# graphdeco-inria/reduced-3dgs

Hardware: AMD Instinct MI355X
Metric: train iters/s (fwd+bwd) + Mpix/s render, 500k Gaussians @1600x1062 (higher is better)
Workload: dtype f32

## Files before the change

include/r3dgs_rasterizer.h:

```cpp
#ifndef R3DGS_RASTERIZER_H
#define R3DGS_RASTERIZER_H

#include <stddef.h>
#include <stdint.h>

#ifdef __cplusplus
extern "C" {
#endif

typedef char* (*r3dgs_alloc_fn)(size_t bytes, void* user);

const char* r3dgs_version(void);

const char* r3dgs_last_error(void);

size_t r3dgs_geometry_bytes(int P);
size_t r3dgs_geometry_bytes_lean(int P);
size_t r3dgs_binning_bytes(int P, int width, int height, int reserve);
size_t r3dgs_image_bytes(int width, int height);
int r3dgs_binning_capacity(int P, int width, int height, size_t bytes);

int r3dgs_mark_visible(int P, const float* means3D, const float* viewmatrix, const float* projmatrix,
                       unsigned char* present, void* stream);

// ... 17 lines not shown
                            int prefiltered, float* out_color, int* out_touched_pixels, float* out_transmittance,
                            int* radii, int calculate_mean_transmittance, int debug, void* stream);

#define R3DGS_PASS_TRUNCATED 1
#define R3DGS_PASS_DEPTH_BUCKET_OVERFLOW 2
int r3dgs_reserve_hint(int P, int width, int height);
int r3dgs_reserve_hint_view(int P, int width, int height, const float* viewmatrix);
long long r3dgs_forward_reserved(char* geom_buffer, char* binning_buffer, char* image_buffer, int reserve, int P,
                                 const int* D, int M, const float* background, int width, int height,
                                 const float* means3D, const float* shs, const float* colors_precomp,
                                 const float* opacities, const float* scales, float scale_modifier,
                                 const float* rotations, const float* cov3D_precomp, const float* viewmatrix,
                                 const float* projmatrix, const float* cam_pos, float tan_fovx, float tan_fovy,
                                 int prefiltered, float* out_color, int* out_touched_pixels, float* out_transmittance,
                                 int* radii, int calculate_mean_transmittance, int debug, void* stream);
long long r3dgs_inference_forward_reserved(char* geom_buffer, char* binning_buffer, char* image_buffer, int reserve,
                                           int P, const int* D, int bandsNum, const int* coeffsNum,
                                           const int* perBandPrimitiveCount, const int* cumSumPrimitiveCount,
                                           const float* background, int width, int height, const float* means3D,
                                           const float* shs, const float* colors_precomp, const float* opacities,
                                           const float* scales, float scale_modifier, const float* rotations,
                                           const float* cov3D_precomp, const float* viewmatrix, const float* projmatrix,
                                           const float* cam_pos, float tan_fovx, float tan_fovy, int prefiltered,
                                           float* out_color, int* out_touched_pixels, float* out_transmittance,
                                           int* radii, int calculate_mean_transmittance, int debug, void* stream);
int r3dgs_pass_query(long long ticket, int wait, int* num_rendered, int* visible, int* reserve, int* flags);
long long r3dgs_reserve_overflow_events(int* last_num_rendered, int* last_reserve);
int r3dgs_pass_pairs(long long ticket, int wait);
int r3dgs_forward_pairs(void);
int r3dgs_set_tight_rects(int on);
int r3dgs_export_rects(int P, char* geom_buffer, unsigned short* rects, void* stream);

int r3dgs_set_tile_order(int on);
int r3dgs_set_sh_cache(int on);
int r3dgs_set_f64_chain(int on);
void r3dgs_forward_hint(int will_backward);

int r3dgs_set_bwd_segments(int on);

int r3dgs_export_tile_order(int P, int R, int width, int height, char* binning_buffer, char* image_buffer,
                            unsigned int* quad_depth, unsigned int* unit_order, void* stream);
int r3dgs_bwd_units_cap(int R, int width, int height);

void r3dgs_reserve_forget(void);
void r3dgs_reserve_forget_view(const float* viewmatrix);

int r3dgs_backward(int P, const int* D, int M, int R, const float* background, int width, int height,
                   const float* means3D, const float* shs, const float* colors_precomp, const float* scales,
                   float scale_modifier, const float* rotations, const float* cov3D_precomp,
                   const float* viewmatrix, const float* projmatrix, const float* campos, float tan_fovx,
                   float tan_fovy, const int* radii, char* geom_buffer, char* binning_buffer, char* image_buffer,
                   const float* dL_dpix, float* dL_dmean2D, float* dL_dconic, float* dL_dopacity, float* dL_dcolor,
                   float* dL_dmean3D, float* dL_dcov3D, float* dL_dsh, float* dL_dscale, float* dL_drot,
                   float lambda_sh_sparsity, int debug, void* stream);

int r3dgs_forward_params(r3dgs_alloc_fn geometryBuffer, void* geometry_user, r3dgs_alloc_fn binningBuffer,
                         void* binning_user, r3dgs_alloc_fn imageBuffer, void* image_user, int P, const int* D, int M,
                         const float* background, int width, int height, const float* means3D, const float* features_dc,
                         const float* features_rest, const float* opacities, const float* scaling_raw,
                         float scale_modifier, const float* rotation_raw, const float* viewmatrix, const float* projmatrix,
                         const float* cam_pos, float tan_fovx, float tan_fovy, int prefiltered, float* out_color,
                         int* out_touched_pixels, float* out_transmittance, int* radii, int calculate_mean_transmittance,
                         int debug, void* stream);
long long r3dgs_forward_params_reserved(char* geom_buffer, char* binning_buffer, char* image_buffer, int reserve, int P,
                                        const int* D, int M, const float* background, int width, int height,
                                        const float* means3D, const float* features_dc, const float* features_rest,
// ... 36 lines not shown
```

reduced-3dgs_amd/csrc/binning.hip:

```cpp
#include <cstdlib>
#include <cstring>
#include <mutex>
#include <string>

#include <rocprim/rocprim.hpp>

#include "depth_sort.h"

namespace r3 {

struct GatherTiles {
    const uint32_t* tiles;
    __host__ __device__ uint32_t operator()(uint32_t id) const { return tiles[id]; }
};

size_t depth_sort_temp_bytes(size_t P)
{
    size_t a = 0, b = 0;
    uint32_t* n = nullptr;
    R3_HIP(rocprim::radix_sort_pairs(nullptr, a, n, n, rocprim::counting_iterator<uint32_t>(0), n, P, 0, 32));
    auto it = rocprim::make_transform_iterator(n, GatherTiles{n});
    R3_HIP(rocprim::inclusive_scan(nullptr, b, it, n, P, rocprim::plus<uint32_t>()));
    return (a > b ? a : b) + 256;
}
// ... 253 lines not shown
__global__ __launch_bounds__(256) void radix_digit_scan_kernel(const RadixArgs* __restrict__ ap)
{
    __shared__ uint32_t s_sum[256];
    const RadixArgs a = *ap;
    const uint32_t nb = (a.hdr->num_pairs + (uint32_t)kRadixBlock - 1u) / (uint32_t)kRadixBlock;
    const uint32_t* row = a.rows + (size_t)blockIdx.x * a.row_stride;
    uint32_t* out = a.base + (size_t)blockIdx.x * a.row_stride;
    uint32_t run = 0;
    for (uint32_t c0 = 0; c0 < nb; c0 += 1024u) {
        const uint32_t i = c0 + threadIdx.x * 4u;
        uint4 v = make_uint4(0u, 0u, 0u, 0u);
        if (i < nb) v = *reinterpret_cast<const uint4*>(row + i);
        if (i + 1 >= nb) v.y = 0u;
        if (i + 2 >= nb) v.z = 0u;
        if (i + 3 >= nb) v.w = 0u;
        const uint32_t mine = v.x + v.y + v.z + v.w;
        const uint32_t incl = block256_inclusive_scan(mine, s_sum);
        const uint32_t b0 = run + incl - mine;
        if (i < nb) *reinterpret_cast<uint4*>(out + i) = make_uint4(b0, b0 + v.x, b0 + v.x + v.y, b0 + v.x + v.y + v.z);
        run += s_sum[0] + s_sum[1] + s_sum[2] + s_sum[3];
    }
    if (threadIdx.x == 0) a.total[blockIdx.x] = run;
}

template <class IO, int BITS>
__device__ __forceinline__ void radix_scatter_block(const RadixArgs& a, uint32_t R, uint32_t blk_id)
{
    constexpr int kWaves = 4, kRounds = kRadixBlock / 256, kBins = 1 << BITS;
    __shared__ uint32_t s_wcount[kWaves][kBins];
    __shared__ uint32_t s_start[kBins];
    __shared__ uint32_t s_off[kWaves][kBins];
    __shared__ uint32_t s_delta[kBins];
    __shared__ typename IO::Reg s_keys[kRadixBlock];
    typedef typename IO::Reg Word;
    const int shift = a.shift;
    const int lane = threadIdx.x & 63, w = threadIdx.x >> 6;
    for (int t = threadIdx.x; t < kWaves * kBins; t += 256) (&s_wcount[0][0])[t] = 0;
    if (w == 0) {
        constexpr int kPer = kBins / 64;
        uint32_t v[kPer], sum = 0;
#pragma unroll
        for (int k = 0; k < kPer; k++) {
            v[k] = a.total[kPer * lane + k];
            sum += v[k];
        }
        uint32_t incl = sum;
        for (int off = 1; off < 64; off <<= 1) {
            const uint32_t up = (uint32_t)__shfl_up((int)incl, off);
            if (lane >= off) incl += up;
        }
        uint32_t run = incl - sum;
#pragma unroll
        for (int k = 0; k < kPer; k++) {
            s_start[kPer * lane + k] = run;
            run += v[k];
        }
    }
    __syncthreads();
    const uint32_t blk = blk_id * (uint32_t)kRadixBlock + (uint32_t)w * (kRadixBlock / kWaves);
    Word key[kRounds];
    uint32_t lrank[kRounds];
#pragma unroll
    for (int r = 0; r < kRounds; r++) {
        const uint32_t i = blk + r * 64u + lane;
        key[r] = i < R ? IO::load(a.in, a.cap, i) : (Word)0;
    }
// ... 19 lines not shown
            v[k] = s_wcount[0][d] + s_wcount[1][d] + s_wcount[2][d] + s_wcount[3][d];
            sum += v[k];
        }
        uint32_t incl = sum;
        for (int off = 1; off < 64; off <<= 1) {
            const uint32_t up = (uint32_t)__shfl_up((int)incl, off);
            if (lane >= off) incl += up;
        }
        uint32_t run = incl - sum;
#pragma unroll
        for (int k = 0; k < kPer; k++) {
            const int d = kPer * lane + k;
            s_delta[d] = s_start[d] + a.base[(size_t)d * a.row_stride + blk_id] - run;
            uint32_t r2 = run;
#pragma unroll
            for (int q = 0; q < kWaves; q++) {
                s_off[q][d] = r2;
                r2 += s_wcount[q][d];
            }
            run += v[k];
        }
    }
    __syncthreads();
#pragma unroll
    for (int r = 0; r < kRounds; r++) {
        if (blk + r * 64u + lane < R) {
            const uint32_t d = (uint32_t)(key[r] >> shift) & (uint32_t)(kBins - 1);
            s_keys[s_off[w][d] + lrank[r]] = key[r];
        }
    }
    __syncthreads();
    const uint32_t base0 = blk_id * (uint32_t)kRadixBlock;
    const uint32_t nvalid = min((uint32_t)kRadixBlock, R - base0);
#pragma unroll
    for (int r = 0; r < kRounds; r++) {
        const uint32_t i = (uint32_t)r * 256u + threadIdx.x;
        if (i < nvalid) {
            const Word k = s_keys[i];
            const uint32_t d = (uint32_t)(k >> shift) & (uint32_t)(kBins - 1);
            IO::store(a.out, a.ids_out, a.cap, i + s_delta[d], k);
        }
    }
}

template <class IO, int BITS>
__global__ __launch_bounds__(256) void radix_scatter_kernel(const RadixArgs* __restrict__ ap)
{
    const RadixArgs a = *ap;
    const uint32_t R = a.hdr->num_pairs;
    for (uint32_t blk = blockIdx.x; blk * (uint32_t)kRadixBlock < R; blk += gridDim.x) {
        radix_scatter_block<IO, BITS>(a, R, blk);
        __syncthreads();
    }
}

template <class IO>
__global__ __launch_bounds__(256) void tile_ranges_kernel(const RangesArgs* __restrict__ ap)
{
    typedef typename IO::Reg Word;
    const RangesArgs a = *ap;
    const int R = (int)a.hdr->num_pairs;
  for (int blk = (int)blockIdx.x; blk * 1024 < R; blk += (int)gridDim.x) {
    const int i0 = (blk * 256 + threadIdx.x) * 4;
    if (i0 >= R) continue;
    unsigned char* __restrict__ pair_flag = a.pair_flag;
    uint32_t* __restrict__ point_list = a.point_list;
    uint2* ranges = a.ranges;
    const int rank_bits = a.rank_bits;
    if (i0 + 4 <= R)
        *reinterpret_cast<uint32_t*>(pair_flag + i0) = 0u;
    else
        for (int k = i0; k < R; k++) pair_flag[k] = 0;
    const int n = min(4, R - i0);
    uint32_t tile[4];
// ... 15 lines not shown
    }
    uint32_t prev = i0 ? IO::tile_at(a.sorted, a.cap, (uint32_t)(i0 - 1), rank_bits) : 0xFFFFFFFFu;
    for (int k = 0; k < n; k++) {
        const uint32_t cur = tile[k];
        const int i = i0 + k;
        if (i == 0)
            ranges[cur].x = 0;
        else if (cur != prev) {
            ranges[prev].y = i;
            ranges[cur].x = i;
        }
        if (i == R - 1) ranges[cur].y = R;
        prev = cur;
    }
  }
}

template <class IO>
static void issue_tile_binning_t(const FwdPlan& p, const FwdPassArgs* a, hipStream_t s)
{
    const PairLayout& l = p.layout;
    const uint32_t nbk = (p.grid_pairs + (uint32_t)kRadixBlock - 1u) / (uint32_t)kRadixBlock;
    const int bins = 1 << l.digit_bits;
    hipLaunchKernelGGL(emit_pairs_kernel<IO>, dim3(nbk), dim3(256), 0, s, &a->emit);
    for (int k = 0; k < l.passes; k++) {
        const RadixArgs* ra = &a->radix[k];
        if (k > 0) hipLaunchKernelGGL(radix_hist_kernel<IO>, dim3(nbk), dim3(256), 0, s, ra);
        hipLaunchKernelGGL(radix_digit_scan_kernel, dim3(bins), dim3(256), 0, s, ra);
        if (l.digit_bits == 7)
            hipLaunchKernelGGL((radix_scatter_kernel<IO, 7>), dim3(nbk), dim3(256), 0, s, ra);
        else
            hipLaunchKernelGGL((radix_scatter_kernel<IO, 8>), dim3(nbk), dim3(256), 0, s, ra);
    }
    hipLaunchKernelGGL(tile_ranges_kernel<IO>, dim3((p.grid_pairs + 1023u) / 1024u), dim3(256), 0, s, &a->ranges);
}

void issue_tile_binning(const FwdPlan& p, const FwdPassArgs* a, hipStream_t s)
{
    if (p.layout.wide == 2)
        issue_tile_binning_t<IoSplit>(p, a, s);
    else if (p.layout.wide == 1)
        issue_tile_binning_t<IoWide>(p, a, s);
    else
        issue_tile_binning_t<IoNarrow>(p, a, s);
}

template <class IO>
__global__ __launch_bounds__(256) void export_keys_kernel(int R, uint32_t cap, int rank_bits, const char* __restrict__ sorted,
                                                          const uint32_t* __restrict__ point_list,
                                                          const uint32_t* __restrict__ depth_key, const GeomHeader* hdr,
                                                          uint64_t* keys)
{
    const int i = blockIdx.x * 256 + threadIdx.x;
    if (i >= R) return;
    if ((uint32_t)i >= hdr->num_pairs) {
        keys[i] = ~(uint64_t)0;
        return;
    }
    keys[i] = ((uint64_t)IO::tile_at(sorted, cap, (uint32_t)i, rank_bits) << 32) | (uint64_t)depth_key[point_list[i]];
}

__global__ __launch_bounds__(256) void export_point_list_kernel(int count, const uint32_t* __restrict__ point_list,
                                                                const GeomHeader* hdr, uint32_t* __restrict__ out)
{
    const int i = blockIdx.x * 256 + threadIdx.x;
    if (i < count && (uint32_t)i < hdr->num_pairs) out[i] = point_list[i];
}
// ... 33 lines not shown
```

reduced-3dgs_amd/csrc/capi.hip:

```cpp
#include "../../include/r3dgs_rasterizer.h"

#include <time.h>

#include <atomic>
#include <random>
#include <chrono>
#include <cmath>
#include <cstddef>
#include <cstdlib>
#include <cstring>
#include <deque>
#include <map>
#include <mutex>
#include <unordered_map>
#include <vector>

#include "common.h"

namespace r3 {
int env_int(const char* env, int dflt, int lo, int hi)
{
    const char* v = getenv(env);
    if (!v) return dflt;
    const int p = atoi(v);
// ... 49 lines not shown
        g_tile_order.store(v);
    }
    return v;
}

std::atomic<int> g_bwd_segments{-1};
int bwd_segments()
{
    int v = g_bwd_segments.load();
    if (v < 0) {
        v = env_int("R3DGS_BWD_SEG", 1, 0, 1);
        g_bwd_segments.store(v);
    }
    return v;
}
std::atomic<int> g_sh_cache{-1};
int sh_derivative_cache()
{
    int v = g_sh_cache.load();
    if (v < 0) {
        v = env_int("R3DGS_SH_CACHE", 1, 0, 1);
        g_sh_cache.store(v);
    }
    return v;
}

std::atomic<int> g_f64_chain{-1};
int f64_chain()
{
    int v = g_f64_chain.load();
    if (v < 0) {
        v = env_int("R3DGS_F64_CHAIN", 1, 0, 1);
        g_f64_chain.store(v);
    }
    return v;
}

bool env_is(const char* name, const char* value)
{
    const char* v = getenv(name);
    return v && std::string(v) == value;
}

size_t cached_depth_temp(size_t P)
{
    static std::mutex mu;
    static std::unordered_map<size_t, size_t> cache;
    std::lock_guard<std::mutex> lk(mu);
    auto it = cache.find(P);
    if (it != cache.end()) return it->second;
    size_t b = depth_sort_temp_bytes(P);
    cache[P] = b;
    return b;
}

template <class Block>
__global__ __launch_bounds__(256) void write_args_kernel(Block* dst, Block v)
{
    static_assert(alignof(Block) == 8 && sizeof(Block) % 4 == 0, "kernarg layout: [dst (8 B)][block]");
#if defined(__HIP_DEVICE_COMPILE__)
    typedef const uint32_t __attribute__((address_space(4))) * KernargWords;
    KernargWords s = (KernargWords)__builtin_amdgcn_kernarg_segment_ptr() + sizeof(Block*) / 4;
    uint32_t* d = reinterpret_cast<uint32_t*>(dst);
    for (uint32_t k = threadIdx.x; k < sizeof(Block) / 4; k += 256) d[k] = s[k];
#endif
    (void)v;
// ... 446 lines not shown
    static const bool generic_env = env_is("R3DGS_DEPTH_SORT", "generic");
    FwdPlan p;
    p.P = c.P;
    p.M = c.M;
    p.W = c.width;
    p.H = c.height;
    p.gx = (c.width + kTile - 1) / kTile;
    p.gy = (c.height + kTile - 1) / kTile;
    p.reserve = reserve;
    p.grid_pairs = grid_pairs_for(reserve);
    p.layout = pair_layout(c.P, (size_t)p.gx * p.gy);
    p.nb = depth_bucket_count((size_t)c.P);
    p.ragged = (c.coeffsNum != nullptr && !c.colors_precomp) ? 1 : 0;
    p.counters = c.calculate_mean_transmittance ? 1 : 0;
    p.fwd_ppl = ppl0 == 3 ? 2 : ppl0;
    p.color_grid = color_grid_env >= 0 ? color_grid_env : std::min(4096, std::max(512, c.P / 512));
    static const int fuse = env_int("R3DGS_COLOR_FUSE", 1, 0, 1);
    static const int split0_env = env_int("R3DGS_COLOR_SPLIT0", -1, 0, 100), split1_env = env_int("R3DGS_COLOR_SPLIT1", -1, 0, 100);
    const bool big = c.P > (1 << 20);
    const int split0 = split0_env >= 0 ? split0_env : 25, split1 = split1_env >= 0 ? split1_env : big ? 25 : 45;
    p.color_fuse = fuse;
    p.color_split[0] = split0;
    p.color_split[1] = split0 + split1 > 100 ? 100 - split0 : split1;
    p.color_split[2] = 100 - p.color_split[0] - p.color_split[1];
    p.generic_depth_sort = (generic_env || c.P >= (1 << 24)) ? 1 : 0;
    static const int in_geom_env = env_int("R3DGS_COLOR_IN_GEOM", -1, -1, 1);
    p.color_in_geom = in_geom_env > 0 ? 1 : 0;
    if (p.color_in_geom) p.color_fuse = 0;
    static const int side_env = env_int("R3DGS_COLOR_STREAM", -1, -1, 1);
    p.color_side = (side_env > 0 && !p.color_in_geom) ? 1 : 0;
    if (p.color_side) p.color_fuse = 0;
    p.tight = tight_rects();
    p.raw_params = c.raw ? 1 : 0;
    return p;
}

void fill_fwd_args(FwdPassArgs& a, const FwdPlan& p, const FwdCall& c, const GeomState& g, const BinState* b,
                   const ImageState& img, PassInfo* info_dev, uint64_t ticket, bool fuse_header)
{
    memset(&a, 0, sizeof(a));
    int* radii = c.radii ? c.radii : g.radii_internal;
    FwdInputs& in = a.pre.in;
    in.P = c.P;
    in.M = c.M;
    in.degrees = c.D;
    in.means3D = c.means3D;
    in.scales = c.scales;
    in.rotations = c.rotations;
    in.opacities = c.opacities;
    in.shs = c.shs;
    in.cov3D_precomp = c.cov3D_precomp;
    in.colors_precomp = c.colors_precomp;
    in.coeffs_num = p.ragged ? c.coeffsNum : nullptr;
    in.per_band_count = p.ragged ? c.perBand : nullptr;
    in.cumsum_count = p.ragged ? c.cumSum : nullptr;
    a.shs_rest = c.raw ? c.shs_rest : nullptr;
    ViewParams& v = a.pre.view;
    v.view = c.viewmatrix;
    v.proj = c.projmatrix;
    v.campos = c.cam_pos;
    v.bg = c.background;
    v.tan_fovx = c.tan_fovx;
    v.tan_fovy = c.tan_fovy;
    v.W = c.width;
    v.H = c.height;
    v.scale_modifier = c.scale_modifier;
// ... 59 lines not shown
        e.hdr = g.header;
        e.order = g.order;
        e.offsets = g.offsets;
        e.block_first = block_first;
        e.rect = g.rect;
        e.rect_sorted = p.generic_depth_sort ? nullptr : g.rect_sorted;
        e.rec = g.rec;
        e.rank_bits = l.rank_bits;
        e.digit_bits = l.digit_bits;
        e.words_out = b->words_a;
        e.cap = p.reserve;
        e.pair_rank = l.wide == 1 ? b->pair_rank : nullptr;
        e.ranges = img.ranges;
        e.n_tiles = (uint32_t)Tn;
        e.radix_rows = b->radix_rows;
        e.row_stride = stride;
        const char* src = b->words_a;
        for (int k = 0; k < l.passes; k++) {
            char* dst = l.wide ? ((k & 1) ? b->words_a : b->words_b) : ((k & 1) ? b->words_c : b->words_b);
            RadixArgs& r = a.radix[k];
            r.hdr = g.header;
            r.in = src;
            r.out = dst;
            r.ids_out = (l.wide == 2 && k == l.passes - 1) ? b->point_list : nullptr;
            r.cap = p.reserve;
            r.shift = l.rank_bits + k * l.digit_bits;
            r.digit_bits = l.digit_bits;
            r.rank_bits = l.rank_bits;
            r.tile_shift = k * l.digit_bits;
            r.rows = b->radix_rows;
            r.base = b->radix_base;
            r.total = b->radix_total + k * kMaxRadixBins;
            r.row_stride = stride;
            src = dst;
        }
        if (src != sorted_words(*b, l)) throw Error("internal: sorted-word buffer mismatch");
        RangesArgs& t = a.ranges;
        t.hdr = g.header;
        t.sorted = src;
        t.cap = p.reserve;
        t.rank_bits = l.rank_bits;
        t.order = nullptr;
        t.point_list = b->point_list;
        t.ranges = img.ranges;
        t.pair_flag = b->pair_flag;
    }
    BlendFwdArgs& f = a.blend;
    f.ranges = img.ranges;
    f.point_list = b ? b->point_list : nullptr;
    f.rec = g.rec;
    f.W = c.width;
    f.H = c.height;
    f.gx = p.gx;
    f.nblocks = (uint32_t)(p.gx * p.gy * (4 / p.fwd_ppl));
    f.bg = c.background;
    f.out_color = c.out_color;
    f.final_T = img.final_T;
    f.n_contrib = img.n_contrib;
    f.touched = p.counters ? c.out_touched_pixels : nullptr;
    f.transmittance = p.counters ? c.out_transmittance : nullptr;
    f.quad_masks = b && keep_quad_masks() ? b->quad_masks : nullptr;
    f.quad_depth = img.quad_depth;
    f.ckpt = ckpt;
    f.hdr = g.header;
}

uint32_t fwd_flags(const FwdPlan& p, const FwdCall& c)
{
    return (uint32_t)p.ragged | ((uint32_t)p.counters << 1) | ((uint32_t)p.fwd_ppl << 2) |
           ((uint32_t)p.layout.wide << 8) | ((uint32_t)(c.colors_precomp != nullptr) << 6) | ((uint32_t)p.color_fuse << 7) |
           ((uint32_t)p.tight << 10) | ((uint32_t)p.color_in_geom << 11) | ((uint32_t)p.color_side << 12) |
           ((uint32_t)p.raw_params << 13);
}

int current_device()
{
    int dev = 0;
    R3_HIP(hipGetDevice(&dev));
    return dev;
}

uint64_t new_ticket(int dev, const FwdCall& c, uint32_t reserve, bool sort_stamp, PassInfo** info_dev)
{
    const uint64_t number = g_next_ticket.fetch_add(1);
    const uint64_t ticket = ((uint64_t)dev << kTicketDevShift) | number;
    InfoRing& ring = info_ring(dev);
    *info_dev = ring.dev + number % kInfoRing;
    std::lock_guard<std::mutex> lk(g_adv.mu);
    g_adv.pending.push_back({ticket, dev, c.P, c.width, c.height, reserve, reinterpret_cast<uintptr_t>(c.viewmatrix), sort_stamp});
    return ticket;
}

bool take_prefer_generic(int dev, const FwdCall& c)
{
    std::lock_guard<std::mutex> lk(g_adv.mu);
    auto it = g_adv.views.find({dev, c.width, c.height});
    if (it == g_adv.views.end() || it->second.prefer_generic <= 0) return false;
    it->second.prefer_generic--;
    return true;
}

size_t geometry_blob_bytes(size_t P, size_t depth_temp, bool lean)
{
    const GeomState g = GeomState::carve(nullptr, P, depth_temp);
    return (size_t)reinterpret_cast<uintptr_t>(lean ? g.lean_end : g.end) + kAlign;
// ... 375 lines not shown
{
    const int before = tight_rects();
    if (on >= 0) g_tight_rects.store(on ? 1 : 0);
    return before;
}

void r3dgs_forward_hint(int will_backward) { g_next_forward_trains = will_backward ? 1 : 0; }

int r3dgs_set_sh_cache(int on)
{
    const int before = sh_derivative_cache();
    if (on >= 0) g_sh_cache.store(on ? 1 : 0);
    return before;
}

int r3dgs_set_f64_chain(int on)
{
    const int before = f64_chain();
    if (on >= 0) g_f64_chain.store(on ? 1 : 0);
    return before;
}

int r3dgs_set_bwd_segments(int on)
{
    const int before = bwd_segments();
    if (on >= 0) g_bwd_segments.store(on ? 1 : 0);
    return before;
}

int r3dgs_set_tile_order(int on)
{
    const int before = heaviest_tiles_first();
    if (on >= 0) g_tile_order.store(on ? 1 : 0);
    return before;
}

int r3dgs_export_rects(int P, char* geom_buffer, unsigned short* rects, void* stream)
{
    return guarded([&]() {
        using namespace r3;
        if (P <= 0) return 0;
        if (!geom_buffer || !rects) throw Error("a required pointer is NULL");
        GeomState geom = GeomState::carve(geom_buffer, (size_t)P, cached_depth_temp((size_t)P));
        R3_HIP(hipMemcpyAsync(rects, geom.rect, sizeof(ushort4) * (size_t)P, hipMemcpyDeviceToDevice,
                              static_cast<hipStream_t>(stream)));
        return 0;
    });
}

void r3dgs_reserve_forget(void)
{
    std::lock_guard<std::mutex> lk(g_adv.mu);
    g_adv.views.clear();
    g_adv.pending.clear();
}

long long r3dgs_reserve_overflow_events(int* last_num_rendered, int* last_reserve)
{
    std::lock_guard<std::mutex> lk(g_adv.mu);
    try {
        harvest_locked();
    } catch (...) {
    }
    if (last_num_rendered) *last_num_rendered = (int)g_adv.last_overflow_rendered;
    if (last_reserve) *last_reserve = (int)g_adv.last_overflow_reserve;
    return (long long)g_adv.overflow_events;
// ... 383 lines not shown
```

reduced-3dgs_amd/csrc/common.h:

```cpp
#pragma once
#include <hip/hip_runtime.h>
#include <stddef.h>
#include <stdint.h>

#include <functional>
#include <stdexcept>
#include <string>

#include "gauss_math.h"
#include "param_math.h"

namespace r3 {

constexpr size_t kAlign = 256;
constexpr int kPairGrad = 9;
#ifndef R3_ACC_STRIDE
#define R3_ACC_STRIDE 12
#endif
#ifndef R3_PAIR_STRIDE
#define R3_PAIR_STRIDE 12
#endif
#ifdef R3_WP_VEC
constexpr int kPieceStride = 12;
#else
constexpr int kPieceStride = 9;
#endif
constexpr int kAccStride = R3_ACC_STRIDE;
constexpr int kPairStride = R3_PAIR_STRIDE;

constexpr int kPreBlockSize = 256;
struct PrePartial {
    uint32_t visible;
    uint32_t num_rendered;
    uint32_t depth_max;
    uint32_t depth_inv_min;
    uint32_t binned;
    uint32_t rendered_ref;
    uint32_t pad[2];
};
static_assert(sizeof(PrePartial) == 32, "two 16-byte loads per partial");
struct GeomHeader {
    uint32_t visible, num_rendered, depth_max, depth_inv_min;
    uint32_t num_pairs;
    uint32_t reserve;
    uint32_t sort_overflow;
    uint32_t binned;
    uint32_t rendered_ref;
    uint32_t sh_cache;
    uint32_t ckpt;
    uint32_t ckpt_thr;
    uint32_t pad[52];
};
static_assert(sizeof(GeomHeader) == 256, "header = 256 B");
inline size_t pre_partials(size_t P) { return (P + kPreBlockSize - 1) / kPreBlockSize; }

struct PassInfo {
    uint32_t seq;
    uint32_t num_rendered;
    uint32_t visible;
    uint32_t reserve;
    uint32_t sort_overflow;
    uint32_t sort_seq;
    uint32_t pairs;
    uint32_t pad;
};
static_assert(sizeof(PassInfo) == 32, "PassInfo = 32 B");

constexpr int kMinDepthBuckets = 1024;
constexpr int kMaxDepthBuckets = 16384;
constexpr int kBucketCap = 4096;
#ifndef R3_HIST_BATCH
#define R3_HIST_BATCH 4096
#endif
constexpr int kHistBatch = R3_HIST_BATCH;
inline size_t depth_hist_per_block(size_t P)
{
    const size_t want = (P + 255) / 256;
    const size_t per = ((want + kHistBatch - 1) / kHistBatch) * kHistBatch;
    return per < (size_t)kHistBatch ? (size_t)kHistBatch : per;
}
int depth_bucket_load();
inline int depth_bucket_count(size_t P)
{
    int nb = kMinDepthBuckets;
// ... 395 lines not shown
    uint32_t* block_first;
    uint32_t block_cap;
};
struct EmitArgs {
    int P, gx;
    const GeomHeader* hdr;
    const uint32_t* order;
    const uint32_t* offsets;
    const uint32_t* block_first;
    const ushort4* rect;
    const ushort4* rect_sorted;
    GRec* rec;
    int rank_bits, digit_bits;
    char* words_out;
    uint32_t cap;
    uint32_t* pair_rank;
    uint2* ranges;
    uint32_t n_tiles;
    uint32_t* radix_rows;
    uint32_t row_stride;
};
struct RadixArgs {
    const GeomHeader* hdr;
    const char* in;
    char* out;
    uint32_t* ids_out;
    uint32_t cap;
    int shift, digit_bits;
    int rank_bits, tile_shift;
    uint32_t* rows;
    uint32_t* base;
    uint32_t* total;
    uint32_t row_stride;
};
struct RangesArgs {
    const GeomHeader* hdr;
    const char* sorted;
    uint32_t cap;
    int rank_bits;
    const uint32_t* order;
    uint32_t* point_list;
    uint2* ranges;
    unsigned char* pair_flag;
};
struct BlendFwdArgs {
    const uint2* ranges;
    const uint32_t* point_list;
    const GRec* rec;
    int W, H, gx;
    uint32_t nblocks;
    const float* bg;
    float* out_color;
    float* final_T;
    uint32_t* n_contrib;
    int* touched;
    float* transmittance;
    unsigned long long* quad_masks;
    uint32_t* quad_depth;
    float4* ckpt;
    const GeomHeader* hdr;
};
struct BlendBwdArgs {
    const uint2* ranges;
    const uint32_t* point_list;
    const GRec* rec;
    const float* final_T;
// ... 47 lines not shown
struct FwdPassArgs {
    PreArgs pre;
    HeaderArgs header;
    DepthArgs depth;
    EmitArgs emit;
    RadixArgs radix[kMaxRadixPasses];
    RangesArgs ranges;
    BlendFwdArgs blend;
    const float* shs_rest;
};
struct BwdPassArgs {
    BlendBwdArgs blend;
    PairReduceArgs reduce;
    PreBwdArgs pre;
};
static_assert(sizeof(FwdPassArgs) <= 3072 && sizeof(BwdPassArgs) <= 3072, "pass blocks travel as by-value kernel arguments");

struct FwdPlan {
    int P, M, W, H, gx, gy;
    uint32_t reserve;
    uint32_t grid_pairs;
    PairLayout layout;
    int nb;
    int ragged, counters;
    int color_in_geom;
    int color_side;
    int fwd_ppl;
    int color_grid;
    int color_fuse;
    int color_split[3];
    int generic_depth_sort;
    int tight;
    int raw_params;
};
struct BwdPlan {
    int P, M, W, H, gx, gy;
    uint32_t reserve, grid_pairs;
    uint32_t units_cap;
    PairLayout layout;
    int bwd_ppl;
    int has_pairs;
    int f64_chain;
    int raw_params;
};

enum Stage { kPre = 0, kDepthSort, kBinning, kBlendFwd, kBlendBwd, kPreBwd, kColor, kBlendBwdKernel, kNumStages };

void issue_preprocess_geom(const FwdPlan& p, FwdPassArgs* dst, const FwdPassArgs& v, hipStream_t s);
void issue_preprocess_color(const FwdPlan& p, const PreArgs* a, hipStream_t s);
void launch_mark_visible(int P, const float* means3D, const float* view, bool* present, hipStream_t s);
void launch_activate_params(int P, const float* scaling_raw, const float* rotation_raw, float* scales, float* rotations,
                            hipStream_t s);

void issue_header_reduce(const HeaderArgs* a, hipStream_t s);
void prepare_depth_bucket_sort(int nb);
void issue_depth_sort_and_color(const FwdPlan& p, const FwdPassArgs* a, hipStream_t s);
void run_generic_depth_sort(int P, GeomState& g, hipStream_t s);
void issue_tile_binning(const FwdPlan& p, const FwdPassArgs* a, hipStream_t s);
const char* sorted_words(const BinState& b, const PairLayout& l);
void launch_export_keys(int P, int R, int cap, size_t n_tiles, const BinState& b, const GeomState& g, uint64_t* keys_out,
                        hipStream_t s);
void launch_export_point_list(int count, const uint32_t* point_list, const GeomHeader* hdr, uint32_t* out, hipStream_t s);

void issue_blend_forward(const FwdPlan& p, const BlendFwdArgs* a, hipStream_t s);
void issue_unit_order(const BwdPlan& p, BwdPassArgs* dst, const BwdPassArgs& v, hipStream_t s);
void issue_blend_backward(const BwdPlan& p, BwdPassArgs* dst, const BwdPassArgs& v, hipStream_t s);
// ... 26 lines not shown
```

reduced-3dgs_amd/csrc/depth_sort.h:

```cpp
#pragma once
#include "common.h"

namespace r3 {

template <class T>
__device__ inline T block256_inclusive_scan(T v, T* s_w)
{
    const int lane = threadIdx.x & 63, w = threadIdx.x >> 6;
    for (int off = 1; off < 64; off <<= 1) {
        const T up = __shfl_up(v, off);
        if (lane >= off) v += up;
    }
    __syncthreads();
    if (lane == 63) s_w[w] = v;
    __syncthreads();
    T add = 0;
    for (int k = 0; k < w; k++) add += s_w[k];
    return v + add;
}

template <int BITS>
__device__ __forceinline__ unsigned long long match_digit(uint32_t d, bool valid)
{
    unsigned long long peers = __ballot(valid);
// ... 77 lines not shown
        s_red[w][2] = acc.depth_max;
        s_red[w][3] = acc.depth_inv_min;
        s_red[w][4] = acc.binned;
        s_red[w][5] = acc.rendered_ref;
    }
    __syncthreads();
    PrePartial out = {0u, 0u, 0u, 0u, 0u, 0u, {0u, 0u}};
    for (int k = 0; k < nw; k++) {
        out.visible += s_red[k][0];
        out.num_rendered += s_red[k][1];
        out.depth_max = max(out.depth_max, s_red[k][2]);
        out.depth_inv_min = max(out.depth_inv_min, s_red[k][3]);
        out.binned += s_red[k][4];
        out.rendered_ref += s_red[k][5];
    }
    __syncthreads();
    return out;
}

__device__ inline void write_header(const HeaderArgs& a, const PrePartial& all)
{
    GeomHeader* hdr = a.hdr;
    hdr->visible = all.visible;
    hdr->num_rendered = all.num_rendered;
    hdr->depth_max = all.depth_max;
    hdr->depth_inv_min = all.depth_inv_min;
    hdr->num_pairs = min(all.num_rendered, a.reserve);
    hdr->reserve = a.reserve;
    hdr->sort_overflow = 0u;
    hdr->binned = all.binned;
    hdr->rendered_ref = all.rendered_ref;
    hdr->sh_cache = a.sh_cache;
    hdr->ckpt = a.ckpt;
    {
        const unsigned long long mean_pct = (unsigned long long)hdr->num_pairs * a.ckpt_factor_pct / (a.n_tiles ? a.n_tiles : 1u);
        const uint32_t thr = (uint32_t)min(mean_pct / 100ull, 0x7FFFFFFFull);
        hdr->ckpt_thr = a.ckpt ? max(thr, 2u << a.ckpt) : 0xFFFFFFFFu;
    }
    volatile PassInfo* info = a.info;
    if (info) {
        info->num_rendered = all.rendered_ref;
        info->pairs = all.num_rendered;
        info->visible = all.visible;
        info->reserve = a.reserve;
        info->sort_overflow = 0u;
        __threadfence_system();
        if (a.stamp_sort) info->sort_seq = a.ticket;
        info->seq = a.ticket;
    }
}

__device__ inline void depth_hist_role(const DepthArgs& a, const HeaderArgs& h, char* smem, int wg)
{
    __shared__ uint32_t s_red[16][6];
    unsigned long long* hist = reinterpret_cast<unsigned long long*>(smem);
    const int P = a.P, nb = a.nb;
    for (int b = threadIdx.x; b <= nb; b += 256) hist[b] = 0;
    uint32_t dmax, dinv;
    if (wg == 0 && threadIdx.x == 0) a.ds->big_count = 0u;
    if (a.fuse_header) {
        const PrePartial all = reduce_partials(h.parts, h.n_parts, s_red);
        if (wg == 0 && threadIdx.x == 0) write_header(h, all);
        dmax = all.depth_max;
        dinv = all.depth_inv_min;
    } else {
        dmax = a.hdr->depth_max;
// ... 625 lines not shown
```

reduced-3dgs_amd/diff_gaussian_rasterization/_C.py:

```python
import ctypes as C
import threading
import weakref
import os

import numpy as np
import torch

_HERE = os.path.dirname(os.path.abspath(__file__))
_LIB_PATH = os.path.join(os.path.dirname(_HERE), "libr3dgs_hip.so")
if os.environ.get("R3DGS_LIB"):
    _v = os.environ["R3DGS_LIB"]
    _LIB_PATH = _v if os.sep in _v else os.path.join(os.path.dirname(_HERE), f"libr3dgs_hip_{_v}.so")
if not os.path.exists(_LIB_PATH):
    raise ImportError(f"{_LIB_PATH} not found: build it with `python reduced-3dgs_amd/build.py` "
                      "(the rasterizer has no CPU or PyTorch fallback)")
_lib = C.CDLL(_LIB_PATH)

_ALLOC = C.CFUNCTYPE(C.c_void_p, C.c_size_t, C.c_void_p)
_vp, _i, _f = C.c_void_p, C.c_int, C.c_float

_lib.r3dgs_version.restype = C.c_char_p
_lib.r3dgs_last_error.restype = C.c_char_p
_lib.r3dgs_geometry_bytes.restype = C.c_size_t
_lib.r3dgs_geometry_bytes.argtypes = [_i]
# ... 15 lines not shown
_lib.r3dgs_inference_forward.argtypes = [_ALLOC, _vp, _ALLOC, _vp, _ALLOC, _vp, _i, _vp, _i, _vp, _vp, _vp] + _FWD_TAIL
_lib.r3dgs_reserve_hint.restype = _i
_lib.r3dgs_reserve_hint.argtypes = [_i, _i, _i]
_lib.r3dgs_reserve_hint_view.restype = _i
_lib.r3dgs_reserve_hint_view.argtypes = [_i, _i, _i, _vp]
_lib.r3dgs_forward_reserved.restype = C.c_longlong
_lib.r3dgs_forward_reserved.argtypes = [_vp, _vp, _vp, _i, _i, _vp, _i] + _FWD_TAIL
_lib.r3dgs_inference_forward_reserved.restype = C.c_longlong
_lib.r3dgs_inference_forward_reserved.argtypes = [_vp, _vp, _vp, _i, _i, _vp, _i, _vp, _vp, _vp] + _FWD_TAIL
_lib.r3dgs_pass_query.restype = _i
_lib.r3dgs_pass_query.argtypes = [C.c_longlong, _i, _vp, _vp, _vp, _vp]
_lib.r3dgs_pass_pairs.restype = _i
_lib.r3dgs_pass_pairs.argtypes = [C.c_longlong, _i]
_lib.r3dgs_forward_pairs.restype = _i
_lib.r3dgs_set_tight_rects.restype = _i
_lib.r3dgs_set_tight_rects.argtypes = [_i]
_lib.r3dgs_forward_hint.restype = None
_lib.r3dgs_forward_hint.argtypes = [_i]
_lib.r3dgs_set_sh_cache.restype = _i
_lib.r3dgs_set_sh_cache.argtypes = [_i]
_lib.r3dgs_reserve_forget_view.restype = None
_lib.r3dgs_reserve_forget_view.argtypes = [C.c_void_p]
_lib.r3dgs_set_f64_chain.restype = _i
_lib.r3dgs_set_f64_chain.argtypes = [_i]
_lib.r3dgs_set_tile_order.restype = _i
_lib.r3dgs_set_tile_order.argtypes = [_i]
_lib.r3dgs_export_tile_order.restype = _i
_lib.r3dgs_export_tile_order.argtypes = [_i, _i, _i, _i, _vp, _vp, _vp, _vp, _vp]
if hasattr(_lib, "r3dgs_bwd_units_cap"):
    _lib.r3dgs_bwd_units_cap.restype = _i
    _lib.r3dgs_bwd_units_cap.argtypes = [_i, _i, _i]
    _lib.r3dgs_set_bwd_segments.restype = _i
    _lib.r3dgs_set_bwd_segments.argtypes = [_i]
_lib.r3dgs_export_rects.restype = _i
_lib.r3dgs_export_rects.argtypes = [_i, _vp, _vp, _vp]
_lib.r3dgs_reserve_overflow_events.restype = C.c_longlong
_lib.r3dgs_reserve_overflow_events.argtypes = [_vp, _vp]
_lib.r3dgs_backward.restype = _i
_lib.r3dgs_backward.argtypes = ([_i, _vp, _i, _i, _vp, _i, _i, _vp, _vp, _vp, _vp, _f, _vp, _vp, _vp, _vp, _vp, _f, _f,
                                 _vp, _vp, _vp, _vp] + [_vp] * 10 + [_f, _i, _vp])
_lib.r3dgs_export_binning.restype = _i
_lib.r3dgs_export_binning.argtypes = [_i, _i, _i, _i, _i] + [_vp] * 10
if hasattr(_lib, "r3dgs_forward_params"):
    _FWD_PARAMS_TAIL = [_vp, _i, _i, _vp, _vp, _vp, _vp, _vp, _f, _vp, _vp, _vp, _vp, _f, _f, _i, _vp, _vp, _vp, _vp, _i, _i, _vp]
    _lib.r3dgs_forward_params.restype = _i
    _lib.r3dgs_forward_params.argtypes = [_ALLOC, _vp, _ALLOC, _vp, _ALLOC, _vp, _i, _vp, _i] + _FWD_PARAMS_TAIL
    _lib.r3dgs_forward_params_reserved.restype = C.c_longlong
    _lib.r3dgs_forward_params_reserved.argtypes = [_vp, _vp, _vp, _i, _i, _vp, _i] + _FWD_PARAMS_TAIL
    _lib.r3dgs_backward_params.restype = _i
    _lib.r3dgs_backward_params.argtypes = ([_i, _vp, _i, _i, _vp, _i, _i, _vp, _vp, _vp, _vp, _f, _vp, _vp, _vp, _vp, _f, _f,
                                            _vp, _vp, _vp, _vp] + [_vp] * 11 + [_f, _i, _vp])
    _lib.r3dgs_activate_params.restype = _i
    _lib.r3dgs_activate_params.argtypes = [_i, _vp, _vp, _vp, _vp, _vp]

_lib.r3dgs_colour_variance_accumulate.restype = _i
_lib.r3dgs_colour_variance_accumulate.argtypes = [_i, _vp, _i, _i] + [_vp] * 12
_lib.r3dgs_min_pixel_size.restype = _i
_lib.r3dgs_min_pixel_size.argtypes = [_i, _i] + [_vp] * 7
_lib.r3dgs_sphere_ellipsoid_intersection.restype = _i
_lib.r3dgs_sphere_ellipsoid_intersection.argtypes = [_i, _i] + [_vp] * 8
_lib.r3dgs_min_redundancy.restype = _i
_lib.r3dgs_min_redundancy.argtypes = [_i, _i] + [_vp] * 5
_lib.r3dgs_kmeans_workspace_bytes.restype = C.c_size_t
_lib.r3dgs_kmeans_workspace_bytes.argtypes = [_i, _i]
_lib.r3dgs_kmeans.restype = _i
_lib.r3dgs_kmeans.argtypes = [_i, _i, _vp, _vp, _f, _i, _vp, _vp, _vp, _vp, _vp]
# ... 755 lines not shown


_tls = threading.local()


def hint_next_forward(will_backward):
    _tls.next_forward_trains = bool(will_backward)


def set_sh_cache(on):
    return bool(_lib.r3dgs_set_sh_cache(int(bool(on))))


def sh_cache():
    return bool(_lib.r3dgs_set_sh_cache(-1))


def set_f64_chain(on):
    return bool(_lib.r3dgs_set_f64_chain(int(bool(on))))


def f64_chain():
    return bool(_lib.r3dgs_set_f64_chain(-1))


def set_tile_order(on):
    return bool(_lib.r3dgs_set_tile_order(int(bool(on))))


def tile_order():
    return bool(_lib.r3dgs_set_tile_order(-1))


def set_bwd_segments(on):
    return bool(_lib.r3dgs_set_bwd_segments(int(bool(on))))


def bwd_segments():
    return bool(_lib.r3dgs_set_bwd_segments(-1))


def export_tile_order(H, W, imageBuffer, P=0, num_rendered=0, binningBuffer=None):
    n = ((W + 15) // 16) * ((H + 15) // 16)
    qd = torch.empty((n, 4), dtype=torch.int32, device=imageBuffer.device)
    out = dict(quad_depth=qd)
    order, R = None, 0
    if binningBuffer is not None and binningBuffer.numel():
        R = (num_rendered.capacity if isinstance(num_rendered, NumRendered) else
             _lib.r3dgs_binning_capacity(int(P), W, H, int(binningBuffer.numel())))
        cap = int(_lib.r3dgs_bwd_units_cap(R, W, H))
        order = torch.empty((cap + 2 * _ORDER_LISTS,), dtype=torch.int32, device=imageBuffer.device)
    with _on_device(imageBuffer.device):
        _check(_lib.r3dgs_export_tile_order(int(P), int(R), W, H, _ptr(binningBuffer) if order is not None else None,
                                            _ptr(imageBuffer), _ptr(qd), _ptr(order) if order is not None else None,
                                            _stream()), "export_tile_order")
    if order is not None:
        o = order.cpu().numpy().astype("int64") & 0xFFFFFFFF
        per = cap // _ORDER_LISTS
        lists = []
        for g in range(_ORDER_LISTS):
            cnt, walk_log2 = int(o[cap + 2 * g]), int(o[cap + 2 * g + 1])
            u = o[g * per:g * per + cnt]
            lists.append(dict(tile=u & 0xFFFFF, segment=(u >> 20) & 63, segments=u >> 26, walk=(1 << walk_log2) if walk_log2 else 0))
        out["lists"] = lists
        out["units"] = {k: np.concatenate([l[k] for l in lists]) for k in ("tile", "segment", "segments")}
    return out
# ... 288 lines not shown
```

Before: 1546.

## Fuse tile range detection into final radix scatter pass

On the last radix pass, the scatter kernel now also writes the point list, clears pair flags, and finds tile range boundaries with atomicMax on the ranges array, using neighbour keys in shared memory. A last-block ticket then converts the inverted start values. This is meant to drop the separate tile_ranges_kernel launch and its full re-read of the sorted pairs. In exchange the scatter kernel does extra atomics, a device-wide fence and ticket, and a final pass over all tiles. The old separate pass can still be selected through an environment variable.

```diff
diff --git a/include/r3dgs_rasterizer.h b/include/r3dgs_rasterizer.h
--- a/include/r3dgs_rasterizer.h
+++ b/include/r3dgs_rasterizer.h
@@ -73,6 +73,7 @@
 int r3dgs_export_rects(int P, char* geom_buffer, unsigned short* rects, void* stream);
 
 int r3dgs_set_tile_order(int on);
+int r3dgs_set_ranges_pass(int on);
 int r3dgs_set_sh_cache(int on);
 int r3dgs_set_f64_chain(int on);
 void r3dgs_forward_hint(int will_backward);
diff --git a/reduced-3dgs_amd/csrc/binning.hip b/reduced-3dgs_amd/csrc/binning.hip
--- a/reduced-3dgs_amd/csrc/binning.hip
+++ b/reduced-3dgs_amd/csrc/binning.hip
@@ -309,6 +309,7 @@
     __shared__ uint32_t s_off[kWaves][kBins];
     __shared__ uint32_t s_delta[kBins];
     __shared__ typename IO::Reg s_keys[kRadixBlock];
+    __shared__ uint32_t s_last;
     typedef typename IO::Reg Word;
     const int shift = a.shift;
     const int lane = threadIdx.x & 63, w = threadIdx.x >> 6;
@@ -394,14 +395,71 @@
     __syncthreads();
     const uint32_t base0 = blk_id * (uint32_t)kRadixBlock;
     const uint32_t nvalid = min((uint32_t)kRadixBlock, R - base0);
+    uint2* const ranges = a.ranges;
+    if (!ranges) {
+#pragma unroll
+        for (int r = 0; r < kRounds; r++) {
+            const uint32_t i = (uint32_t)r * 256u + threadIdx.x;
+            if (i < nvalid) {
+                const Word k = s_keys[i];
+                const uint32_t d = (uint32_t)(k >> shift) & (uint32_t)(kBins - 1);
+                IO::store(a.out, a.ids_out, a.cap, i + s_delta[d], k);
+            }
+        }
+        return;
+    }
+    const int rank_bits = a.rank_bits;
+    uint32_t* __restrict__ point_list = a.point_list;
+    {
+        static_assert(kRadixBlock == 256 * 8, "eight pair flags per thread");
+        unsigned char* flags = a.pair_flag + base0 + threadIdx.x * 8u;
+        const uint32_t f0 = threadIdx.x * 8u;
+        if (f0 + 8u <= nvalid)
+            *reinterpret_cast<uint2*>(flags) = make_uint2(0u, 0u);
+        else
+            for (uint32_t k = f0; k < nvalid; k++) a.pair_flag[base0 + k] = 0;
+    }
 #pragma unroll
     for (int r = 0; r < kRounds; r++) {
         const uint32_t i = (uint32_t)r * 256u + threadIdx.x;
         if (i < nvalid) {
             const Word k = s_keys[i];
             const uint32_t d = (uint32_t)(k >> shift) & (uint32_t)(kBins - 1);
-            IO::store(a.out, a.ids_out, a.cap, i + s_delta[d], k);
-        }
+            const uint32_t pos = i + s_delta[d];
+            IO::store(a.out, a.ids_out, a.cap, pos, k);
+            if (!IO::kIdsApart) point_list[pos] = (uint32_t)(k & ((((Word)1) << rank_bits) - 1));
+        }
+    }
+#pragma unroll 1
+    for (uint32_t i = threadIdx.x; i < nvalid; i += 256u) {
+        const Word k = s_keys[i];
+        const uint32_t d = (uint32_t)(k >> shift) & (uint32_t)(kBins - 1);
+        const uint32_t pos = i + s_delta[d];
+        const uint32_t tile = (uint32_t)(k >> rank_bits);
+        const Word kp = s_keys[i ? i - 1u : 0u], kn = s_keys[i + 1u < nvalid ? i + 1u : i];
+        const bool has_prev = i > 0u && ((uint32_t)(kp >> shift) & (uint32_t)(kBins - 1)) == d;
+        const bool has_next = i + 1u < nvalid && ((uint32_t)(kn >> shift) & (uint32_t)(kBins - 1)) == d;
+        const uint32_t tprev = (uint32_t)(kp >> rank_bits);
+        if (!has_prev || tprev != tile) atomicMax(&ranges[tile].x, ~pos);
+        if (has_prev && tprev != tile) atomicMax(&ranges[tprev].y, pos);
+        if (!has_next) atomicMax(&ranges[tile].y, pos + 1u);
+    }
+    __threadfence();
+    __syncthreads();
+    if (threadIdx.x == 0) {
+        const uint32_t n_blocks = (R + (uint32_t)kRadixBlock - 1u) / (uint32_t)kRadixBlock;
+        s_last = atomicAdd(a.ticket, 1u) == n_blocks - 1u ? 1u : 0u;
+    }
+    __syncthreads();
+    if (s_last) {
+        __threadfence();
+        unsigned long long* cells = reinterpret_cast<unsigned long long*>(ranges);
+#pragma unroll 4
+        for (uint32_t t = threadIdx.x; t < a.n_tiles; t += 256u) {
+            const unsigned long long c = __hip_atomic_load(cells + t, __ATOMIC_RELAXED, __HIP_MEMORY_SCOPE_AGENT);
+            if ((uint32_t)(c >> 32)) ranges[t].x = ~(uint32_t)c;
+        }
+        if (threadIdx.x == 0) *a.ticket = 0u;
     }
 }
 
@@ -483,7 +541,7 @@
         else
             hipLaunchKernelGGL((radix_scatter_kernel<IO, 8>), dim3(nbk), dim3(256), 0, s, ra);
     }
-    hipLaunchKernelGGL(tile_ranges_kernel<IO>, dim3((p.grid_pairs + 1023u) / 1024u), dim3(256), 0, s, &a->ranges);
+    if (p.ranges_pass) hipLaunchKernelGGL(tile_ranges_kernel<IO>, dim3((p.grid_pairs + 1023u) / 1024u), dim3(256), 0, s, &a->ranges);
 }
 
 void issue_tile_binning(const FwdPlan& p, const FwdPassArgs* a, hipStream_t s)
diff --git a/reduced-3dgs_amd/csrc/capi.hip b/reduced-3dgs_amd/csrc/capi.hip
--- a/reduced-3dgs_amd/csrc/capi.hip
+++ b/reduced-3dgs_amd/csrc/capi.hip
@@ -105,6 +105,17 @@
     if (v < 0) {
         v = env_int("R3DGS_F64_CHAIN", 1, 0, 1);
         g_f64_chain.store(v);
+    }
+    return v;
+}
+
+std::atomic<int> g_ranges_pass{-1};
+int ranges_pass()
+{
+    int v = g_ranges_pass.load();
+    if (v < 0) {
+        v = env_int("R3DGS_RANGES_PASS", 0, 0, 1);
+        g_ranges_pass.store(v);
     }
     return v;
 }
@@ -617,6 +628,7 @@
     if (p.color_side) p.color_fuse = 0;
     p.tight = tight_rects();
     p.raw_params = c.raw ? 1 : 0;
+    p.ranges_pass = ranges_pass();
     return p;
 }
 
@@ -742,6 +754,13 @@
             r.base = b->radix_base;
             r.total = b->radix_total + k * kMaxRadixBins;
             r.row_stride = stride;
+            if (k == l.passes - 1 && !p.ranges_pass) {
+                r.point_list = b->point_list;
+                r.ranges = img.ranges;
+                r.pair_flag = b->pair_flag;
+                r.ticket = &g.header->ranges_ticket;
+                r.n_tiles = (uint32_t)Tn;
+            }
             src = dst;
         }
         if (src != sorted_words(*b, l)) throw Error("internal: sorted-word buffer mismatch");
@@ -780,7 +799,7 @@
     return (uint32_t)p.ragged | ((uint32_t)p.counters << 1) | ((uint32_t)p.fwd_ppl << 2) |
            ((uint32_t)p.layout.wide << 8) | ((uint32_t)(c.colors_precomp != nullptr) << 6) | ((uint32_t)p.color_fuse << 7) |
            ((uint32_t)p.tight << 10) | ((uint32_t)p.color_in_geom << 11) | ((uint32_t)p.color_side << 12) |
-           ((uint32_t)p.raw_params << 13);
+           ((uint32_t)p.raw_params << 13) | ((uint32_t)p.ranges_pass << 14);
 }
 
 int current_device()
@@ -1222,6 +1241,13 @@
 {
     const int before = heaviest_tiles_first();
     if (on >= 0) g_tile_order.store(on ? 1 : 0);
+    return before;
+}
+
+int r3dgs_set_ranges_pass(int on)
+{
+    const int before = ranges_pass();
+    if (on >= 0) g_ranges_pass.store(on ? 1 : 0);
     return before;
 }
 
diff --git a/reduced-3dgs_amd/csrc/common.h b/reduced-3dgs_amd/csrc/common.h
--- a/reduced-3dgs_amd/csrc/common.h
+++ b/reduced-3dgs_amd/csrc/common.h
@@ -49,7 +49,8 @@
     uint32_t sh_cache;
     uint32_t ckpt;
     uint32_t ckpt_thr;
-    uint32_t pad[52];
+    uint32_t ranges_ticket;
+    uint32_t pad[51];
 };
 static_assert(sizeof(GeomHeader) == 256, "header = 256 B");
 inline size_t pre_partials(size_t P) { return (P + kPreBlockSize - 1) / kPreBlockSize; }
@@ -511,6 +512,11 @@
     uint32_t* base;
     uint32_t* total;
     uint32_t row_stride;
+    uint32_t* point_list;
+    uint2* ranges;
+    unsigned char* pair_flag;
+    uint32_t* ticket;
+    uint32_t n_tiles;
 };
 struct RangesArgs {
     const GeomHeader* hdr;
@@ -624,6 +630,7 @@
     int generic_depth_sort;
     int tight;
     int raw_params;
+    int ranges_pass;
 };
 struct BwdPlan {
     int P, M, W, H, gx, gy;
diff --git a/reduced-3dgs_amd/csrc/depth_sort.h b/reduced-3dgs_amd/csrc/depth_sort.h
--- a/reduced-3dgs_amd/csrc/depth_sort.h
+++ b/reduced-3dgs_amd/csrc/depth_sort.h
@@ -133,6 +133,7 @@
     hdr->rendered_ref = all.rendered_ref;
     hdr->sh_cache = a.sh_cache;
     hdr->ckpt = a.ckpt;
+    hdr->ranges_ticket = 0u;
     {
         const unsigned long long mean_pct = (unsigned long long)hdr->num_pairs * a.ckpt_factor_pct / (a.n_tiles ? a.n_tiles : 1u);
         const uint32_t thr = (uint32_t)min(mean_pct / 100ull, 0x7FFFFFFFull);
diff --git a/reduced-3dgs_amd/diff_gaussian_rasterization/_C.py b/reduced-3dgs_amd/diff_gaussian_rasterization/_C.py
--- a/reduced-3dgs_amd/diff_gaussian_rasterization/_C.py
+++ b/reduced-3dgs_amd/diff_gaussian_rasterization/_C.py
@@ -71,6 +71,9 @@
     _lib.r3dgs_bwd_units_cap.argtypes = [_i, _i, _i]
     _lib.r3dgs_set_bwd_segments.restype = _i
     _lib.r3dgs_set_bwd_segments.argtypes = [_i]
+if hasattr(_lib, "r3dgs_set_ranges_pass"):
+    _lib.r3dgs_set_ranges_pass.restype = _i
+    _lib.r3dgs_set_ranges_pass.argtypes = [_i]
 _lib.r3dgs_export_rects.restype = _i
 _lib.r3dgs_export_rects.argtypes = [_i, _vp, _vp, _vp]
 _lib.r3dgs_reserve_overflow_events.restype = C.c_longlong
@@ -892,6 +895,14 @@
     return bool(_lib.r3dgs_set_tile_order(-1))
 
 
+def set_ranges_pass(on):
+    return bool(_lib.r3dgs_set_ranges_pass(int(bool(on))))
+
+
+def ranges_pass():
+    return bool(_lib.r3dgs_set_ranges_pass(-1))
+
+
 def set_bwd_segments(on):
     return bool(_lib.r3dgs_set_bwd_segments(int(bool(on))))
 
```

New measurement: 1239. -19.9%, worse.
